# aws/karpenter-core

Measured on NVIDIA B200. Metric: pods scheduled/sec (Scheduler.Solve), higher is better.
Workload: dtype int64

## Files before the change

karpenter-core_b200/csrc/ksched.cu:

```cuda
#include <cuda_runtime.h>
#include <nccl.h>
#include <stdint.h>

#include <algorithm>
#include <chrono>
#include <cstdio>
#include <cstdlib>
#include <cstring>
#include <cub/cub.cuh>
#include <string>
#include <mutex>
#include <vector>

#include "ksched.h"
#include "reqmask.cuh"
#include "launch.cuh"

using ksched::KeyMeta;
using ksched::Req;

#define CUDA_TRY(h, expr)                                                                         \
  do {                                                                                            \
    cudaError_t _e = (expr);                                                                      \
    if (_e != cudaSuccess) {                                                                      \
// ... 697 lines not shown
        for (uint32_t f = g.filter_begin; f < g.filter_end && f < (uint32_t)pb->n_filter_terms; ++f)
          if (((pb->filter_terms[f].meta >> KSCHED_META_PRESENT_SHIFT) & 0xFFFF) == 0) x.has_filter = 0;
        x.max_skew = g.max_skew; x.host_row = host_row[ct.group];
        relx[e] = x;
      }
      CUDA_TRY(h, upload_vec(h, h->d_relx, relx));
    }
    CUDA_TRY(h, upload_vec(h, h->d_grp_host_total0, host_total));
    CUDA_TRY(h, upload_vec(h, h->d_grp_cnt0, cnt));
    CUDA_TRY(h, upload_vec(h, h->d_grp_registered0, registered));
    CUDA_TRY(h, h->d_grp_host0.ensure((size_t)std::max(nh, 1) * stride));
    CUDA_TRY(h, cudaMemsetAsync(h->d_grp_host0.ptr, 0, (size_t)std::max(nh, 1) * stride * sizeof(uint16_t), h->stream));
    if (NE > 0 && nh > 0) {
      CUDA_TRY(h, cudaMemcpy2DAsync(h->d_grp_host0.ptr, stride * sizeof(uint16_t), host.data(), (size_t)NE * sizeof(uint16_t), (size_t)NE * sizeof(uint16_t),
                                    (size_t)nh, cudaMemcpyHostToDevice, h->stream));
      h->tm.h2d_bytes += (int64_t)nh * NE * 2;
    }
    CUDA_TRY(h, cudaStreamSynchronize(h->stream));
    CUDA_TRY(h, h->d_grp_host_total.ensure(std::max(NG, 1)));
    CUDA_TRY(h, h->d_grp_cnt.ensure((size_t)std::max(NG, 1) * 64));
    CUDA_TRY(h, h->d_grp_registered.ensure(std::max(NG, 1)));
    CUDA_TRY(h, h->d_grp_host.ensure((size_t)std::max(nh, 1) * stride));
  }
  const size_t p1 = (size_t)std::max(P, 1);
  CUDA_TRY(h, h->d_order.ensure(p1)); CUDA_TRY(h, h->d_idx_tmp.ensure(p1)); CUDA_TRY(h, h->d_pod_pos.ensure(p1));
  CUDA_TRY(h, h->d_k_cpu.ensure(p1)); CUDA_TRY(h, h->d_k_mem.ensure(p1)); CUDA_TRY(h, h->d_k_tie.ensure(p1)); CUDA_TRY(h, h->d_k_tmp.ensure(p1));
  CUDA_TRY(h, h->d_rows.ensure(p1 * KSCHED_ROW_WORDS));
  CUDA_TRY(h, h->d_F.ensure(p1 * V * W32));
  CUDA_TRY(h, h->d_best.ensure(p1));
  CUDA_TRY(h, h->d_Fclass.ensure((size_t)std::max(NC, 1) * V * W32));
  CUDA_TRY(h, h->d_best_class.ensure((size_t)std::max(NC, 1)));
  CUDA_TRY(h, h->d_relax.ensure(p1)); CUDA_TRY(h, h->d_assign.ensure(p1)); CUDA_TRY(h, h->d_place_seq.ensure(p1));
  CUDA_TRY(h, h->d_queue.ensure(p1 + 1)); CUDA_TRY(h, h->d_last_len.ensure(p1)); CUDA_TRY(h, h->d_last_epoch.ensure(p1));
  const size_t mn = (size_t)MAXN;
  CUDA_TRY(h, h->d_nn_tmpl.ensure(mn)); CUDA_TRY(h, h->d_nn_count.ensure(mn)); CUDA_TRY(h, h->d_nn_tb.ensure(mn));
  CUDA_TRY(h, h->d_nn_req.ensure(8 * mn)); CUDA_TRY(h, h->d_nn_req_present.ensure(mn));
  CUDA_TRY(h, h->d_nn_vals.ensure(16 * mn)); CUDA_TRY(h, h->d_nn_meta.ensure(mn));
  CUDA_TRY(h, h->d_nn_opts.ensure((size_t)W32 * mn)); CUDA_TRY(h, h->d_nn_hp.ensure(mn));
  CUDA_TRY(h, h->d_ov_key.ensure(mn)); CUDA_TRY(h, h->d_ov_q.ensure(4 * mn)); CUDA_TRY(h, h->d_ov_bound.ensure(4 * mn)); CUDA_TRY(h, h->d_ov_bound2.ensure(4 * mn));
  CUDA_TRY(h, h->d_ov_node.ensure(mn)); CUDA_TRY(h, h->d_ov_flags.ensure(mn));
  CUDA_TRY(h, h->d_ov_absorbed.ensure(mn)); CUDA_TRY(h, h->d_ov_rejected.ensure(mn));
  {
    const size_t nfc = (size_t)std::max(NC, 1) * V;
    CUDA_TRY(h, h->d_fc_state.ensure(nfc)); CUDA_TRY(h, h->d_fc_dom.ensure(nfc)); CUDA_TRY(h, h->d_fc_front_state.ensure(nfc)); CUDA_TRY(h, h->d_fc_bound.ensure(nfc * 4)); CUDA_TRY(h, h->d_fc_bound2.ensure(nfc * 4));
    CUDA_TRY(h, h->d_fc_opts.ensure(nfc * W32));
    CUDA_TRY(h, h->d_fc_vals.ensure(nfc * KSCHED_MAX_KEYS)); CUDA_TRY(h, h->d_fc_meta.ensure(nfc)); CUDA_TRY(h, h->d_fc_q.ensure(nfc * KSCHED_MAX_RES));
    CUDA_TRY(h, h->d_fc_qp.ensure(nfc));
    const size_t nfd = kFreshMemoSlots;
    CUDA_TRY(h, h->d_fd_state.ensure(nfd)); CUDA_TRY(h, h->d_fd_dom.ensure(nfd)); CUDA_TRY(h, h->d_fd_fc.ensure(nfd)); CUDA_TRY(h, h->d_fd_meta.ensure(nfd));
    CUDA_TRY(h, h->d_fd_vals.ensure(nfd * KSCHED_MAX_KEYS)); CUDA_TRY(h, h->d_fd_opts.ensure(nfd * W32));
    CUDA_TRY(h, h->d_fd_bound.ensure(nfd * 4)); CUDA_TRY(h, h->d_fd_bound2.ensure(nfd * 4));
  }
  CUDA_TRY(h, h->d_remaining.ensure((size_t)V * KSCHED_MAX_RES));
  CUDA_TRY(h, h->d_counters.ensure(48));
  {
    size_t need = 0, n2 = 0;
    cub::DeviceRadixSort::SortPairs(nullptr, need, (uint64_t*)nullptr, (uint64_t*)nullptr, (uint32_t*)nullptr, (uint32_t*)nullptr, (int)p1, 0, 64, h->stream);
    n2 = need;
    CUDA_TRY(h, h->d_cub_tmp.ensure(n2 + 256));
    h->cub_tmp_bytes = n2 + 256;
  }
  CUDA_TRY(h, cudaStreamSynchronize(h->stream));
  h->uploaded = true;
  h->sorted = false;
  return KSCHED_OK;
}

static int run_sort(ksched_handle* h) {
  const int P = h->n_pods;
  if (P == 0) return KSCHED_OK;
  const int threads = 256, blocks = (P + threads - 1) / threads;
  if (h->sort1_bits > 0) {
    sort_key1_kernel<<<blocks, threads, 0, h->stream>>>(P, h->d_cls_rank.ptr, h->d_pod_class.ptr, h->d_ts.ptr, h->d_uid_rank.ptr, h->sort1_ts_min,
                                                        h->sort1_ts_bits, h->sort1_uid_bits, h->d_k_tie.ptr, h->d_idx_tmp.ptr);
    size_t tmp1 = h->cub_tmp_bytes;
    CUDA_TRY(h, cub::DeviceRadixSort::SortPairs(h->d_cub_tmp.ptr, tmp1, h->d_k_tie.ptr, h->d_k_tmp.ptr, h->d_idx_tmp.ptr, h->d_order.ptr, P, 0, h->sort1_bits,
                                                h->stream));
    const int gblocks1 = std::min((P + 7) / 8, 148 * 8);
    gather_rows_kernel<<<gblocks1, 256, 0, h->stream>>>(P, h->d_classes.ptr, h->d_pod_class.ptr, h->d_order.ptr, h->d_rows.ptr);
    h->tm.sort_launches = 3;
    h->sorted = true;
    return KSCHED_OK;
  }
  sort_keys_kernel<<<blocks, threads, 0, h->stream>>>(P, h->d_classes.ptr, h->d_pod_class.ptr, h->d_ts.ptr, h->d_uid_rank.ptr, h->d_k_cpu.ptr,
                                                      h->d_k_mem.ptr, h->d_k_tie.ptr, h->d_order.ptr);
  size_t tmp = h->cub_tmp_bytes;
  uint32_t *ia = h->d_order.ptr, *ib = h->d_idx_tmp.ptr;
  CUDA_TRY(h, cub::DeviceRadixSort::SortPairs(h->d_cub_tmp.ptr, tmp, h->d_k_tie.ptr, h->d_k_tmp.ptr, ia, ib, P, 0, 64, h->stream));
  gather_u64_kernel<<<blocks, threads, 0, h->stream>>>(P, h->d_k_mem.ptr, ib, h->d_k_tie.ptr);
  tmp = h->cub_tmp_bytes;
  CUDA_TRY(h, cub::DeviceRadixSort::SortPairs(h->d_cub_tmp.ptr, tmp, h->d_k_tie.ptr, h->d_k_tmp.ptr, ib, ia, P, 0, 64, h->stream));
  gather_u64_kernel<<<blocks, threads, 0, h->stream>>>(P, h->d_k_cpu.ptr, ia, h->d_k_tie.ptr);
  tmp = h->cub_tmp_bytes;
  CUDA_TRY(h, cub::DeviceRadixSort::SortPairs(h->d_cub_tmp.ptr, tmp, h->d_k_tie.ptr, h->d_k_tmp.ptr, ia, ib, P, 0, 64, h->stream));
  CUDA_TRY(h, cudaMemcpyAsync(h->d_order.ptr, ib, (size_t)P * sizeof(uint32_t), cudaMemcpyDeviceToDevice, h->stream));
  const int gblocks = std::min((P + 7) / 8, 148 * 8);
  gather_rows_kernel<<<gblocks, 256, 0, h->stream>>>(P, h->d_classes.ptr, h->d_pod_class.ptr, h->d_order.ptr, h->d_rows.ptr);
  h->tm.sort_launches = 7;
  h->sorted = true;
  return KSCHED_OK;
}

static void fill_k1(ksched_handle* h, K1Params& k1) {
  k1.cat = h->cat;
  k1.rows = reinterpret_cast<const uint64_t*>(h->d_classes.ptr);
  k1.n_pods = h->n_classes;
  k1.itype_sets = h->d_itype_sets.ptr;
// ... 64 lines not shown
  if (h->n_pods == 0) return KSCHED_OK;
  const int RW = h->cat.n_templates * h->cat.W32;
  const int nblk = (h->n_pods + 31) / 32;
  const int blocks = std::max(1, std::min(148 * 8, (nblk + 7) / 8));
  feasibility_kernel<<<blocks, 256, 0, h->stream>>>(h->d_rows.ptr, h->n_pods, h->n_classes, RW, h->d_Fclass.ptr, h->d_best_class.ptr, h->d_F.ptr,
                                                    h->d_best.ptr);
  CUDA_TRY(h, cudaGetLastError());
  h->tm.feasibility_launches = 2;
  const long long C = (long long)h->cat.n_templates * h->cat.n_types;
  h->tm.feasibility_bytes = (long long)h->n_pods * 256 + C * 256 + (long long)h->n_pods * C / 8;
  return KSCHED_OK;
}

struct ResetSeg { void* dst; const void* src; unsigned long long bytes; };
struct ResetTable { int n; ResetSeg seg[30]; };
__global__ void reset_kernel(ResetTable t) {
  const size_t tid = (size_t)blockIdx.x * blockDim.x + threadIdx.x, nth = (size_t)gridDim.x * blockDim.x;
  for (int q = 0; q < t.n; ++q) {
    const ResetSeg sg = t.seg[q];
    const size_t n16 = sg.bytes / 16;
    uint4* d = static_cast<uint4*>(sg.dst);
    const uint4* sv = static_cast<const uint4*>(sg.src);
    for (size_t i = tid; i < n16; i += nth) d[i] = sv ? sv[i] : make_uint4(0, 0, 0, 0);
    unsigned char* db = static_cast<unsigned char*>(sg.dst);
    const unsigned char* sb = static_cast<const unsigned char*>(sg.src);
    for (size_t i = n16 * 16 + tid; i < sg.bytes; i += nth) db[i] = sb ? sb[i] : 0;
  }
}

static int reset_state(ksched_handle* h, const int64_t* d_remaining_src = nullptr, void* also_zero = nullptr, size_t also_zero_bytes = 0) {
  const int P = h->n_pods, NE = std::max(h->n_existing, 1), NG = std::max(h->n_groups, 1);
  CUDA_TRY(h, h->d_cls_cursor.ensure((size_t)std::max(h->n_classes, 1)));
  ResetTable t{};
  auto add = [&](void* dst, const void* src, size_t bytes) { if (bytes) t.seg[t.n++] = ResetSeg{dst, src, (unsigned long long)bytes}; };
  add(h->d_pod_class.ptr, h->d_pod_class0.ptr, (size_t)P * 4);
  add(h->d_relax.ptr, nullptr, (size_t)std::max(P, 1) * 4);
  add(h->d_ex_req.ptr, h->d_ex_req0.ptr, (size_t)8 * NE * 8);
  add(h->d_ex_req_present.ptr, h->d_ex_req_present0.ptr, (size_t)NE * 4);
  add(h->d_ex_vals.ptr, h->d_ex_vals0.ptr, (size_t)16 * NE * 8);
  add(h->d_ex_meta.ptr, h->d_ex_meta0.ptr, (size_t)NE * 8);
  add(h->d_ex_hp.ptr, h->d_ex_hp0.ptr, (size_t)NE * 8);
  add(h->d_ex_closed.ptr, nullptr, (size_t)NE);
  add(h->d_cls_cursor.ptr, nullptr, (size_t)std::max(h->n_classes, 1) * 4);
  if (h->have_volumes) add(h->d_ex_vol.ptr, h->d_ex_vol0.ptr, (size_t)h->n_existing * sizeof(ksched_node_volumes));
  add(h->d_grp_cnt.ptr, h->d_grp_cnt0.ptr, (size_t)NG * 64 * 4);
  add(h->d_grp_registered.ptr, h->d_grp_registered0.ptr, (size_t)NG * 8);
  add(h->d_grp_host_total.ptr, h->d_grp_host_total0.ptr, (size_t)NG * 4);
  add(h->d_grp_active.ptr, h->d_grp_active0.ptr, (size_t)NG);
  add(h->d_grp_min_slot.ptr, nullptr, (size_t)NG * 4);
  const size_t hs = (size_t)std::max(h->n_hostgroups, 1) * ((size_t)h->n_existing + h->max_new);
  add(h->d_grp_host.ptr, h->d_grp_host0.ptr, hs * 2);
  if (d_remaining_src)
    add(h->d_remaining.ptr, d_remaining_src, (size_t)h->cat.n_templates * KSCHED_MAX_RES * 8);
  add(h->d_counters.ptr, nullptr, 48 * sizeof(long long));
  add(h->d_fc_state.ptr, nullptr, (size_t)std::max(h->n_classes, 1) * h->cat.n_templates);
  add(h->d_fc_front_state.ptr, nullptr, (size_t)std::max(h->n_classes, 1) * h->cat.n_templates);
  add(h->d_fd_state.ptr, nullptr, (size_t)kFreshMemoSlots);
  add(also_zero, nullptr, also_zero_bytes);
  if (!d_remaining_src) {
    std::vector<int64_t> rem((size_t)h->cat.n_templates * KSCHED_MAX_RES);
    for (int v = 0; v < h->cat.n_templates; ++v)
      for (int r = 0; r < KSCHED_MAX_RES; ++r) rem[(size_t)v * KSCHED_MAX_RES + r] = h->h_templates[v].remaining[r];
    CUDA_TRY(h, cudaMemcpyAsync(h->d_remaining.ptr, rem.data(), rem.size() * 8, cudaMemcpyHostToDevice, h->stream));
    CUDA_TRY(h, cudaStreamSynchronize(h->stream));
  }
  reset_kernel<<<148 * 2, 256, 0, h->stream>>>(t);
  CUDA_TRY(h, cudaGetLastError());
  return KSCHED_OK;
}

static std::mutex g_k2_mu;
static cudaEvent_t g_k2_done[64] = {};

static int run_pack(ksched_handle* h) {
  K2Params& k2 = h->k2_host;
  k2.cat = h->cat;
  PackState& s = k2.st;
  s.relx = h->d_relx.ptr;
  s.classes = h->d_classes.ptr; s.groups = h->d_groups.ptr; s.class_topo = h->d_class_topo.ptr; s.filter_terms = h->d_filter_terms.ptr;
  s.itype_sets = h->d_itype_sets.ptr; s.itype_complement = h->d_itype_comp.ptr; s.hostname_reqs = h->d_hostname_reqs.ptr;
  s.order = h->d_order.ptr; s.rows = h->d_rows.ptr; s.F = h->d_F.ptr; s.best = h->d_best.ptr;
  s.pod_pos = h->d_pod_pos.ptr; s.use_F = h->world == 1 ? 1 : 0;
  s.n_pods = h->n_pods; s.n_classes = h->n_classes; s.n_existing = h->n_existing; s.n_groups = h->n_groups; s.max_new = h->max_new;
  for (int r = 0; r < KSCHED_MAX_RES; ++r) s.min_req[r] = h->min_req[r];
  s.pod_class = h->d_pod_class.ptr; s.relax_level = h->d_relax.ptr; s.assign = h->d_assign.ptr; s.place_seq = h->d_place_seq.ptr;
  s.queue = h->d_queue.ptr; s.last_len = h->d_last_len.ptr; s.last_epoch = h->d_last_epoch.ptr;
  s.ex_req = h->d_ex_req.ptr; s.ex_avail = h->d_ex_avail.ptr; s.ex_req_present = h->d_ex_req_present.ptr; s.ex_avail_present = h->d_ex_avail_present.ptr;
  s.ex_vals = h->d_ex_vals.ptr; s.ex_meta = h->d_ex_meta.ptr; s.ex_taintset = h->d_ex_taintset.ptr; s.ex_itype = h->d_ex_itype.ptr;
  s.ex_hp = h->d_ex_hp.ptr; s.ex_closed = h->d_ex_closed.ptr;
  s.cls_cursor = h->d_cls_cursor.ptr;
  s.cls_vol = h->have_volumes ? h->d_cls_vol.ptr : nullptr; s.ex_vol = h->have_volumes ? h->d_ex_vol.ptr : nullptr;
  for (int d = 0; d < KSCHED_MAX_VOLUME_DRIVERS; ++d) s.vol_mask[d] = h->vol_mask[d];
  s.nn_tmpl = h->d_nn_tmpl.ptr; s.nn_count = h->d_nn_count.ptr; s.nn_tb = h->d_nn_tb.ptr; s.nn_req = h->d_nn_req.ptr;
  s.nn_req_present = h->d_nn_req_present.ptr;
  s.nn_vals = h->d_nn_vals.ptr; s.nn_meta = h->d_nn_meta.ptr; s.nn_opts = h->d_nn_opts.ptr; s.nn_hp = h->d_nn_hp.ptr;
  s.ov_key = h->d_ov_key.ptr; s.ov_q = h->d_ov_q.ptr; s.ov_bound = h->d_ov_bound.ptr; s.ov_bound2 = h->d_ov_bound2.ptr; s.ov_node = h->d_ov_node.ptr; s.ov_flags = h->d_ov_flags.ptr;
  s.fc_state = h->d_fc_state.ptr; s.fc_opts = h->d_fc_opts.ptr; s.fc_bound = h->d_fc_bound.ptr; s.fc_bound2 = h->d_fc_bound2.ptr; s.fc_dom = h->d_fc_dom.ptr; s.fc_front_state = h->d_fc_front_state.ptr;
  s.fc_vals = h->d_fc_vals.ptr; s.fc_meta = h->d_fc_meta.ptr; s.fc_q = h->d_fc_q.ptr; s.fc_qp = h->d_fc_qp.ptr;
  s.ov_absorbed = h->d_ov_absorbed.ptr; s.ov_rejected = h->d_ov_rejected.ptr;
  s.fd_cap = kFreshMemoSlots; s.fd_state = h->d_fd_state.ptr; s.fd_fc = h->d_fd_fc.ptr; s.fd_meta = h->d_fd_meta.ptr; s.fd_vals = h->d_fd_vals.ptr;
  s.fd_opts = h->d_fd_opts.ptr; s.fd_bound = h->d_fd_bound.ptr; s.fd_bound2 = h->d_fd_bound2.ptr; s.fd_dom = h->d_fd_dom.ptr;
  s.count_visited = h->count_visited;
  s.stop_new_nodes = h->stop_new_nodes;
  s.grp_cnt = h->d_grp_cnt.ptr; s.grp_registered = h->d_grp_registered.ptr; s.grp_host = h->d_grp_host.ptr;
  s.grp_host_row = h->d_grp_host_row.ptr; s.grp_host_total = h->d_grp_host_total.ptr; s.remaining = h->d_remaining.ptr;
  s.grp_active = h->d_grp_active.ptr; s.grp_min_slot = h->d_grp_min_slot.ptr;
  s.counters = h->d_counters.ptr;
// ... 60 lines not shown
    ncclResult_t r = ncclAllReduce(h->d_best.ptr, h->d_best.ptr, (size_t)h->n_pods, ncclUint64, ncclMin, h->comm, h->stream);
    if (r != ncclSuccess) { h->err = std::string("ncclAllReduce: ") + ncclGetErrorString(r); return KSCHED_ERR_NCCL; }
  }
  CUDA_TRY(h, cudaEventRecord(h->ev[3], h->stream));
  if ((rc = run_pack(h)) != KSCHED_OK) return rc;
  CUDA_TRY(h, cudaEventRecord(h->ev[4], h->stream));
  CUDA_TRY(h, cudaStreamSynchronize(h->stream));
  CUDA_TRY(h, cudaGetLastError());
  h->tm.sort_us = ev_us(h->ev[0], h->ev[1]);
  h->tm.feasibility_us = ev_us(h->ev[1], h->ev[2]);
  h->tm.allreduce_us = ev_us(h->ev[2], h->ev[3]);
  h->tm.pack_us = ev_us(h->ev[3], h->ev[4]);
  h->tm.total_us = ev_us(h->ev[0], h->ev[4]);
  return KSCHED_OK;
}

int ksched_run_feasibility_only(ksched_handle* h, int do_flush, float* elapsed_us) {
  if (!h || !h->uploaded) return KSCHED_ERR_INVALID;
  CUDA_TRY(h, cudaSetDevice(h->device));
  int rc;
  if (!h->sorted) {
    CUDA_TRY(h, cudaMemcpyAsync(h->d_pod_class.ptr, h->d_pod_class0.ptr, (size_t)h->n_pods * 4, cudaMemcpyDeviceToDevice, h->stream));
    if ((rc = run_sort(h)) != KSCHED_OK) return rc;
  }
  CUDA_TRY(h, cudaEventRecord(h->ev[7], h->stream));
  if ((rc = run_class_feasibility(h)) != KSCHED_OK) return rc;
  if (do_flush && (rc = flush_l2(h)) != KSCHED_OK) return rc;
  CUDA_TRY(h, cudaEventRecord(h->ev[5], h->stream));
  if ((rc = run_feasibility(h)) != KSCHED_OK) return rc;
  CUDA_TRY(h, cudaEventRecord(h->ev[6], h->stream));
  CUDA_TRY(h, cudaStreamSynchronize(h->stream));
  CUDA_TRY(h, cudaGetLastError());
  if (elapsed_us) *elapsed_us = ev_us(h->ev[5], h->ev[6]);
  h->tm.feasibility_us = ev_us(h->ev[5], h->ev[6]);
  h->tm.class_feasibility_us = ev_us(h->ev[7], h->ev[5]);
  return KSCHED_OK;
}

#ifdef KSCHED_PROFILE_PACK
static void print_pack_profile(const long long* counters) {
  fprintf(stderr, "[pack profile] generic: topo=%lld existing=%lld eval=%lld commit=%lld fresh=%lld fail=%lld | fastblock=%lld genericcall=%lld | "
                  "n_generic=%lld inflight_placed=%lld fresh_steps=%lld failures=%lld paths[rej,cached,row,dyn,cachedempty]=%lld,%lld,%lld,%lld,%lld steps=%lld\n",
          counters[8], counters[9], counters[10], counters[11], counters[12], counters[13], counters[14], counters[15], counters[17], counters[18],
          counters[19], counters[20], counters[21], counters[22], counters[23], counters[24], counters[25], counters[5]);
  fprintf(stderr, "[pack profile] fresh: decide=%lld words=%lld commit=%lld rest=%lld | in-flight verify=%lld\n", counters[26], counters[27], counters[28],
          counters[12], counters[29]);
  fprintf(stderr, "[pack profile] in-flight commit: winner+barrier=%lld record=%lld rest=%lld\n", counters[30], counters[31], counters[11]);
  fprintf(stderr, "[pack profile] class_run: calls=%lld pods=%lld bails=%lld ineligible=%lld cycles=%lld\n", counters[40], counters[41], counters[42], counters[43],
          counters[14]);
  fprintf(stderr, "[pack profile] mask run steps=%lld with >1 admissible domain=%lld round-able=%lld (counters shared with generic n/fresh: ignore there)\n", counters[18], counters[19], counters[17]);
  fprintf(stderr, "[pack profile] mask run: build cycles=%lld (refused %lld) loop cycles=%lld pods=%lld entries=%lld\n", counters[38], counters[47], counters[6], counters[7], counters[16]);
  fprintf(stderr, "[pack profile] class_run without mask-key spread: cycles=%lld pods=%lld level+fill iterations=%lld (fill %lld) fresh=%lld per-pod=%lld | with: cycles=%lld pods=%lld fresh=%lld per-pod=%lld\n",
          counters[32], counters[33], counters[34], counters[46], counters[35], counters[44], counters[36], counters[37], counters[39], counters[45]);
}
#endif

int ksched_download(ksched_handle* h, const ksched_problem* pb, ksched_result* res) {
  if (!h || !pb || !res || !h->uploaded) return KSCHED_ERR_INVALID;
  CUDA_TRY(h, cudaSetDevice(h->device));
  const int P = h->n_pods, NE = h->n_existing, MAXN = h->max_new, W32 = h->cat.W32, W64 = h->W64, V = h->cat.n_templates;
  long long counters[48];
  CUDA_TRY(h, cudaMemcpyAsync(counters, h->d_counters.ptr, sizeof counters, cudaMemcpyDeviceToHost, h->stream));
  CUDA_TRY(h, cudaStreamSynchronize(h->stream));
#ifdef KSCHED_PROFILE_PACK
  print_pack_profile(counters);
#endif
  if (counters[4] != 0) {
    h->err = counters[4] == KSCHED_ERR_OVERFLOW ? "new-node capacity exceeded" : "a pod is constrained by more topology groups than the kernel supports";
    return (int)counters[4];
  }
  const int n_new = (int)counters[0];
  h->tm.d2h_bytes = (int64_t)sizeof counters + (int64_t)P * 4 * ((res->assign != nullptr) + (res->relax_level != nullptr) + (res->place_seq != nullptr)) +
                    (int64_t)n_new * (1 + 4 + 4 + 8 + 64 + 128 + (int64_t)W32 * 4) + (res->existing_reqs ? (int64_t)NE * 136 : 0) +
                    (res->launch ? (int64_t)n_new * (int64_t)sizeof(ksched_launch_choice) : 0) +
                    (res->feasibility ? (int64_t)P * V * W32 * 4 + (int64_t)P * 4 : 0) + (res->best_column ? (int64_t)P * 12 : 0);
  res->n_new_nodes = n_new;
  res->n_unscheduled = (int)counters[1];
  res->nodes_visited = counters[2];
  res->add_calls = counters[3];
  h->tm.pack_steps = counters[5];
  if (res->assign) CUDA_TRY(h, cudaMemcpyAsync(res->assign, h->d_assign.ptr, (size_t)P * 4, cudaMemcpyDeviceToHost, h->stream));
  if (res->relax_level) CUDA_TRY(h, cudaMemcpyAsync(res->relax_level, h->d_relax.ptr, (size_t)P * 4, cudaMemcpyDeviceToHost, h->stream));
  if (res->place_seq) CUDA_TRY(h, cudaMemcpyAsync(res->place_seq, h->d_place_seq.ptr, (size_t)P * 4, cudaMemcpyDeviceToHost, h->stream));
  if (n_new > 0 && res->new_nodes && res->new_node_types) {
    std::vector<uint8_t> tmpl(n_new);
    std::vector<int32_t> count(n_new);
    std::vector<int64_t> req((size_t)8 * n_new);
    std::vector<uint32_t> reqp(n_new), opts((size_t)W32 * n_new);
    std::vector<uint64_t> vals((size_t)16 * n_new), meta(n_new);
    CUDA_TRY(h, cudaMemcpyAsync(tmpl.data(), h->d_nn_tmpl.ptr, n_new, cudaMemcpyDeviceToHost, h->stream));
    CUDA_TRY(h, cudaMemcpyAsync(count.data(), h->d_nn_count.ptr, (size_t)n_new * 4, cudaMemcpyDeviceToHost, h->stream));
    CUDA_TRY(h, cudaMemcpyAsync(reqp.data(), h->d_nn_req_present.ptr, (size_t)n_new * 4, cudaMemcpyDeviceToHost, h->stream));
    CUDA_TRY(h, cudaMemcpyAsync(meta.data(), h->d_nn_meta.ptr, (size_t)n_new * 8, cudaMemcpyDeviceToHost, h->stream));
    CUDA_TRY(h, cudaMemcpy2DAsync(req.data(), (size_t)n_new * 8, h->d_nn_req.ptr, (size_t)MAXN * 8, (size_t)n_new * 8, 8, cudaMemcpyDeviceToHost, h->stream));
    CUDA_TRY(h, cudaMemcpy2DAsync(vals.data(), (size_t)n_new * 8, h->d_nn_vals.ptr, (size_t)MAXN * 8, (size_t)n_new * 8, 16, cudaMemcpyDeviceToHost, h->stream));
    CUDA_TRY(h, cudaMemcpy2DAsync(opts.data(), (size_t)n_new * 4, h->d_nn_opts.ptr, (size_t)MAXN * 4, (size_t)n_new * 4, W32, cudaMemcpyDeviceToHost, h->stream));
    CUDA_TRY(h, cudaStreamSynchronize(h->stream));
    for (int n = 0; n < n_new; ++n) {
      ksched_new_node& o = res->new_nodes[n];
      std::memset(&o, 0, sizeof o);
      o.template_index = tmpl[n];
      o.pod_count = count[n];
      o.requests_present = reqp[n];
      for (int r = 0; r < 8; ++r) o.requests[r] = req[(size_t)r * n_new + n];
      for (int k = 0; k < 16; ++k) o.reqs.values[k] = vals[(size_t)k * n_new + n];
      o.reqs.meta = meta[n];
      uint32_t* dst = reinterpret_cast<uint32_t*>(res->new_node_types + (size_t)n * W64);
      for (int w = 0; w < W32; ++w) dst[w] = opts[(size_t)w * n_new + n];
      if (W32 & 1) dst[W32] = 0;
    }
  }
  if (res->launch && n_new > 0) {
    if (!h->cat.offer_keys) { h->err = "ksched_result.launch needs ksched_catalog.offering_keys"; return KSCHED_ERR_INVALID; }
    CUDA_TRY(h, h->d_launch.ensure((size_t)n_new));
// ... 255 lines not shown
```

karpenter-core_b200/csrc/pack_kernel.cuh:

```cuda
#pragma once

namespace {

constexpr int kActCap = 1280;
constexpr int kHotRes = 4;

struct HotSmem {
  unsigned long long key[kActCap];
  long long q[kHotRes][kActCap];
  long long bound[kHotRes][kActCap];
  long long bound2[kHotRes][kActCap];
  int node[kActCap];
  unsigned short flags[kActCap];
  unsigned absorbed[kActCap];
  unsigned rejected[kActCap];
  unsigned long long nn_last[kActCap];
};

struct Hot {
  HotSmem* sm;
  unsigned long long* ov_key;
  long long* ov_q;
  long long* ov_bound;
  long long* ov_bound2;
// ... 1170 lines not shown
    io->add_calls = add_calls;
  }
}

constexpr int kRunHost = 4;
constexpr int kRunMask = 2;
constexpr int kRunDom = 16;
constexpr int kTopoCap = 768;
constexpr int kRunVariants = 4;
constexpr int kRunW32 = 64;
constexpr int kRunWarps = kPackThreads / 32;
constexpr int kRunChunk = 128;
constexpr unsigned kRoomSlow = 0xFFFFu, kRoomMax = 0x7FFEu, kRpDead = 0x80000000u;
constexpr size_t kRunArrayBytes = (size_t)kTopoCap * (kRunMask * 4 + kRunHost * 2) + (size_t)kActCap * 4;

struct RunVariant {
  uint32_t opts[kRunW32];
  uint64_t vals[KSCHED_MAX_KEYS];
  uint64_t meta;
  long long q[KSCHED_MAX_RES];
  long long b1[kHotRes], b2[kHotRes];
  uint32_t qp;
  uint32_t rp;
  unsigned short fl;
  uint8_t dom[kRunMask];
};
struct RunCtx {
  uint32_t cls;
  int eligible;
  int n_host, n_mask, n_var, var_next;
  int tomb;
  int h_row[kRunHost], h_group[kRunHost], h_lim[kRunHost];
  int h_inc[kRunHost];
  uint8_t h_times[kRunHost];
  int m_group[kRunMask], m_skew[kRunMask];
  uint8_t m_key[kRunMask], m_self[kRunMask], m_rec[kRunMask], m_wk[kRunMask];
  uint32_t m_registered[kRunMask], m_neutral[kRunMask], m_tallow[kRunMask];
  int32_t cnt[kRunWarps][kRunMask][kRunDom];
  unsigned long long red_key[2][32];
  unsigned red_pay[2][32];
  uint32_t q_pod[2][kRunChunk], q_cls[2][kRunChunk];
  int32_t q_node[2][kRunChunk];
  int q_end[2];
  int lv_cnt[2];
  int lv_fill[2];
  RunVariant var[kRunVariants];
};
__shared__ RunCtx g_rc;

constexpr int kM1Dom = 8;
constexpr int kM1Lists = kM1Dom + 1;
constexpr int kM1Lv = 12;
constexpr uint16_t kM1None = 0xFFFF;
struct M1Ctx {
  uint16_t tl[kM1Lv][kM1Lists];
  uint16_t head[kM1Lists];
  uint16_t ap[kM1Lv][kM1Lists];
  uint16_t ae[kM1Lv][kM1Lists];
  int bcnt[kM1Lv * kM1Lists];
  int bad;
  int out_adv, out_reason, out_tick, out_n_new, out_n_active;
  int n_fresh;
  uint32_t fr[kRunChunk];
};
__shared__ M1Ctx g_m1;

struct RunIO {
  int qi, head, qlen, tick, seq, n_active, n_new, parity;
  long long add_calls;
  int placed;
  int status;
  int fresh_valid, fresh_a;
  uint32_t fresh_cls;
};
__shared__ RunIO g_rio;

__device__ __forceinline__ int run_pick(uint32_t cand, const int32_t* cn) {
  int d = __ffs(cand) - 1;
  cand &= cand - 1;
  int32_t best = cn[d];
  while (cand) {
    const int e = __ffs(cand) - 1;
    cand &= cand - 1;
    if (cn[e] < best) { best = cn[e]; d = e; }
  }
  return d;
}
__device__ __noinline__ unsigned run_room(const HotSmem* hs, int a, const long long* req, uint32_t res, int RH) {
  const unsigned short fl = hs->flags[a];
  const uint32_t qp = ((fl >> 1) & 0xF) | res;
  long long best = 0;
  bool inexact_ok = true;
  for (int f = 0; f < 2; ++f) {
    if (f == 1 && !(fl & kFlTwo)) break;
    long long rf = kRoomMax;
    for (int r = 0; r < RH; ++r) {
      if (!((qp >> r) & 1)) continue;
      const long long slack = (f ? hs->bound2[r][a] : hs->bound[r][a]) - hs->q[r][a];
      if (req[r] > 0) {
        const long long k = slack < req[r] ? 0 : slack / req[r];
        rf = k < rf ? k : rf;
      } else if (slack < 0) rf = 0;
    }
    if (f == 0) inexact_ok = rf > 0;
    best = rf > best ? rf : best;
  }
// ... 351 lines not shown
            int lv = La - 1;
            while (m1.tl[lv][L] == kM1None) --lv;
            const int pred = m1.tl[lv][L];
            m1_nxt[a] = m1_nxt[pred];
            m1_nxt[pred] = (uint16_t)a;
            if (m1.tl[La][L] == kM1None) m1.tl[La][L] = (uint16_t)a;
            if (pred == h) { n1 = a; nk = ak; nr = ar; }
            if (pred == tcur) { bn = a; bnc = La; }
          }
        };
        auto insert_back1 = [&](int a, unsigned long long ak, uint32_t ar) {
          const int hl = h >= 0 ? (int)(hk >> 32) : 0x7fffffff;
          if (hl > 1) {
            m1_nxt[a] = h >= 0 ? (uint16_t)h : kM1None;
            m1.tl[1][L] = (uint16_t)a;
            tcur = a; bn = h; bnc = hl;
            n1 = h; nk = hk; nr = hr;
            h = a; hk = ak; hr = ar;
          } else if (hl == 1) {
            m1_nxt[a] = bn >= 0 ? (uint16_t)bn : kM1None;
            m1_nxt[tcur] = (uint16_t)a;
            m1.tl[1][L] = (uint16_t)a;
            if (tcur == h) { n1 = a; nk = ak; nr = ar; }
            tcur = a;
          } else {
            int lv = 1;
            while (m1.tl[lv][L] == kM1None) --lv;
            const int pred = m1.tl[lv][L];
            m1_nxt[a] = m1_nxt[pred];
            m1_nxt[pred] = (uint16_t)a;
            m1.tl[1][L] = (uint16_t)a;
            if (pred == h) { n1 = a; nk = ak; nr = ar; }
            if (pred == tcur) { bn = a; bnc = 1; }
          }
        };
        auto pop_head = [&](int c) {
          h = n1; hk = nk; hr = nr;
          n1 = -1; nk = ~0ull; nr = 0;
          if (h >= 0) {
            n1 = nxt_of(h);
            if (n1 >= 0) { nk = hs->key[n1]; nr = rpv[n1]; }
          }
          if (h < 0 || (int)(hk >> 32) != c) {
            m1.tl[c][L] = kM1None;
            level_state();
          }
        };
        const bool rounds = m_rec0 && m_bias0 == 0;
        int li = i, ltick = tick, lnew = n_new, lact = n_active, nfr = 0;
        int i_end = rc.q_end[buf];
        if (i + qlen < i_end) i_end = i + qlen;
        int reason = 0;
        const int slack = m_bias0 < -(1 << 30) ? (1 << 30) : -m_bias0;
        while (li < i_end) {
          const int mn = __reduce_min_sync(FULL, valid ? cnt_d : INT32_MAX);
          const bool allowed = valid && cnt_d - mn <= slack;
          const unsigned okm = __ballot_sync(FULL, allowed);
          const bool cand_ok = L < kM1Dom ? allowed : (L == kM1Dom && okm != 0);
          const unsigned long long key = cand_ok ? hk : ~0ull;
          const unsigned long long wkey = warp_min_u64(key);
#ifdef KSCHED_PROFILE_PACK
          {
            const unsigned have = __ballot_sync(FULL, L < kM1Dom && allowed && h >= 0);
            const unsigned long long ukey = __shfl_sync(FULL, hk, kM1Dom);
            unsigned long long mx = (L < kM1Dom && allowed && h >= 0) ? hk : 0ull;
            for (int o = 16; o; o >>= 1) { const unsigned long long t = __shfl_xor_sync(FULL, mx, o); mx = t > mx ? t : mx; }
            const int na = __popc(okm);
            if (L == 0 && na > 1 && have == okm && ukey > mx && i_end - li >= na) s.counters[17] += 1;
            if (L == 0) s.counters[18] += 1;
            if (L == 0 && na > 1) s.counters[19] += 1;
          }
#endif
          if (rounds) {
            const int na = __popc(okm);
            if (na > 1 && i_end - li >= na) {
              const bool act = L < kM1Dom && allowed;
              const bool hd = act && h >= 0;
              const unsigned hv = __ballot_sync(FULL, hd), fv = okm & ~hv;
              const bool bad_l = hd && ((hr & 0xFFFF) == kRoomSlow || (int)(hk >> 32) + 1 >= kM1Lv);
              const unsigned long long ukey = __shfl_sync(FULL, hk, kM1Dom);
              const unsigned hi = hd ? (unsigned)(hk >> 32) : 0u;
              const unsigned mhi = __reduce_max_sync(FULL, hi);
              const unsigned mlo = __reduce_max_sync(FULL, (hd && hi == mhi) ? (unsigned)hk : 0u);
              const unsigned long long mx = ((unsigned long long)mhi << 32) | mlo;
              int vi_l = -1;
              const int nf = __popc(fv);
              bool fresh_ok = true;
              if (fv) {
                const bool fl = act && h < 0;
                if (fl) for (int v2 = 0; v2 < rc.n_var && vi_l < 0; ++v2) if (rc.var[v2].dom[0] == L) vi_l = v2;
                fresh_ok = ukey == ~0ull && (fv & ~rc.m_tallow[0]) == 0 && !__any_sync(FULL, fl && vi_l < 0) && lnew + nf <= MAXN &&
                           lact + nf <= kActCap && lact + nf <= kTopoCap;
                for (int j = 0; j < n_host; ++j) fresh_ok = fresh_ok && rc.h_lim[j] >= 0;
              }
              if (fresh_ok && !__any_sync(FULL, bad_l) && (hv == 0 || ukey > mx)) {
                int rank = 0;
                for (unsigned m = hv; m; m &= m - 1) {
                  const unsigned long long k2 = __shfl_sync(FULL, hk, __ffs(m) - 1);
                  rank += k2 < hk;
                }
                bool closed_l = false;
                if (hd) {
                  const int a = h;
                  const uint32_t rp = hr;
                  const int c = (int)(hk >> 32);
                  const int mytick = ltick + rank;
                  pop_head(c);
// ... 8 lines not shown
                  const unsigned long long nkey = order_key(c + 1, -(mytick + 1));
                  unsigned long long skey = nkey;
                  rc.q_node[buf][li + rank] = -(a + 2);
                  if ((rp2 & 0xFFFF) == 0) {
                    const int placed = (rp2 >> 16) & 0x7FFF;
                    long long nq[kHotRes], cb1[kHotRes], cb2[kHotRes];
#pragma unroll
                    for (int r = 0; r < kHotRes; ++r) { nq[r] = hs->q[r][a] + placed * p_req[r]; cb1[r] = hs->bound[r][a]; cb2[r] = hs->bound2[r][a]; }
                    const unsigned short fl = (unsigned short)(hs->flags[a] | ((p_res & 0xF) << 1));
                    if (node_closed(nq, min_req, RH, cb1, cb2, fl)) {
                      skey = ~0ull;
                      hs->nn_last[a] = ((unsigned long long)(unsigned)(c + 1) << 32) | (unsigned)(-(mytick + 1));
                      closed_l = true;
                    }
                  }
                  hs->key[a] = skey;
                  rpv[a] = rp2;
                  if ((rp2 & 0xFFFF) != 0 && !(rp2 & kRpDead)) insert_front(a, c + 1, nkey, rp2);
                  ++cnt_d;
                } else if (act) {
                  const RunVariant& v = rc.var[vi_l];
                  const int idx = __popc(fv & ((1u << L) - 1u));
                  const int n = lnew + idx, a = lact + idx;
                  const int mytick = ltick + __popc(hv) + idx;
                  for (int j = 0; j < n_host; ++j) {
                    const int times = rc.h_times[j];
                    hc[j * kTopoCap + a] = (uint16_t)times;
                    if (times) s.grp_host[(size_t)rc.h_row[j] * hstride + NE + n] = (uint16_t)times;
                  }
                  const unsigned long long fkey = order_key(1, mytick + 1);
                  hs->key[a] = fkey;
#pragma unroll
                  for (int r = 0; r < kHotRes; ++r) { hs->q[r][a] = v.q[r]; hs->bound[r][a] = v.b1[r]; hs->bound2[r][a] = v.b2[r]; }
                  hs->node[a] = n;
                  hs->flags[a] = v.fl;
                  hs->absorbed[a] = simple ? cls : KSCHED_NONE;
                  hs->rejected[a] = KSCHED_NONE;
                  rpv[a] = v.rp;
                  rc.q_node[buf][li + __popc(hv) + idx] = NE + n;
                  zv[a] = (1u << L) | (3u << 16);
                  m1.fr[nfr + idx] = (uint32_t)a | ((uint32_t)vi_l << 16);
                  if ((v.rp & 0xFFFF) != 0 && !(v.rp & kRpDead)) insert_back1(a, fkey, v.rp);
                  ++cnt_d;
                }
                if (nf && L < n_host && rc.h_times[L]) rc.h_inc[L] = rc.h_inc[L] + nf;
                const unsigned tb = __ballot_sync(FULL, closed_l);
                if (L == 0 && tb) rc.tomb = rc.tomb + __popc(tb);
                lnew += nf;
                lact += nf;
                nfr += nf;
                ltick += na;
                li += na;
                __syncwarp();
                continue;
              }
            }
          }
          if (wkey != ~0ull) {
            const int wl = __ffs(__ballot_sync(FULL, key == wkey)) - 1;
            const int a = __shfl_sync(FULL, h, wl);
            const uint32_t rp = __shfl_sync(FULL, hr, wl);
            if ((rp & 0xFFFF) == kRoomSlow) { reason = 1; break; }
            int d = wl;
            const bool pin = wl == kM1Dom;
            if (pin) {
              const int mc = __reduce_min_sync(FULL, allowed ? cnt_d : INT32_MAX);
              d = __ffs(__ballot_sync(FULL, allowed && cnt_d == mc)) - 1;
              if (!((rc.m_neutral[0] >> d) & 1) || !((zv[a] & (1u << 17)) || rc.m_wk[0])) { reason = 1; break; }
            }
            const int c = (int)(wkey >> 32);
            if (L == wl) pop_head(c);
            uint32_t rp2 = rp - 1 + (1u << 16);
            bool dead_l = false;
            if (L < n_host) {
              const int times = rc.h_times[L];
              const int old = hc[L * kTopoCap + a];
              const int now = old + times > 0xFFFF ? 0xFFFF : old + times;
              if (times) hc[L * kTopoCap + a] = (uint16_t)now;
              dead_l = now > rc.h_lim[L];
            }
            if (n_host > 0 && __any_sync(FULL, dead_l)) rp2 |= kRpDead;
            const unsigned long long nkey = order_key(c + 1, -(ltick + 1));
            if (L == 0) {
              unsigned long long skey = nkey;
              if (pin) {
                const int n = hs->node[a], k = rc.m_key[0];
                zv[a] = (1u << d) | (3u << 16);
                s.nn_vals[(size_t)k * MAXN + n] = 1ull << d;
                atomicOr(reinterpret_cast<unsigned long long*>(&s.nn_meta[n]), 1ull << (KSCHED_META_PRESENT_SHIFT + k));
                atomicAnd(reinterpret_cast<unsigned long long*>(&s.nn_meta[n]), ~(1ull << (KSCHED_META_COMPLEMENT_SHIFT + k)));
              }
              rc.q_node[buf][li] = -(a + 2);
              if ((rp2 & 0xFFFF) == 0) {
                const int placed = (rp2 >> 16) & 0x7FFF;
                long long nq[kHotRes], cb1[kHotRes], cb2[kHotRes];
#pragma unroll
                for (int r = 0; r < kHotRes; ++r) { nq[r] = hs->q[r][a] + placed * p_req[r]; cb1[r] = hs->bound[r][a]; cb2[r] = hs->bound2[r][a]; }
                const unsigned short fl = (unsigned short)(hs->flags[a] | ((p_res & 0xF) << 1));
                if (node_closed(nq, min_req, RH, cb1, cb2, fl)) {
                  skey = ~0ull;
                  hs->nn_last[a] = ((unsigned long long)(unsigned)(c + 1) << 32) | (unsigned)(-(ltick + 1));
                  rc.tomb = rc.tomb + 1;
                }
              }
              hs->key[a] = skey;
              rpv[a] = rp2;
            }
            if ((rp2 & 0xFFFF) != 0 && !(rp2 & kRpDead)) {
              if (c + 1 >= kM1Lv) reason = 2;
              else if (L == d) insert_front(a, c + 1, nkey, rp2);
            }
            if (m_rec0 && L == d) ++cnt_d;
            ++ltick;
            ++li;
            __syncwarp();
            if (reason == 2) break;
          } else {
            if (lnew >= MAXN || lact >= kActCap || lact >= kTopoCap || rc.n_var == 0) { reason = 1; break; }
            bool ok = true;
            for (int j = 0; j < n_host; ++j) ok = ok && rc.h_lim[j] >= 0;
            const unsigned cand = rc.m_tallow[0] & okm;
            if (!ok || !cand) { reason = 1; break; }
            const bool in_c = (cand >> L) & 1;
            const int mc = __reduce_min_sync(FULL, in_c ? cnt_d : INT32_MAX);
            const int fd = __ffs(__ballot_sync(FULL, in_c && cnt_d == mc)) - 1;
            int vi = -1;
            for (int v2 = 0; v2 < rc.n_var && vi < 0; ++v2) if (rc.var[v2].dom[0] == fd) vi = v2;
            if (vi < 0) { reason = 1; break; }
            const RunVariant& v = rc.var[vi];
            const int n = lnew, a = lact;
            if (L < n_host) {
              const int times = rc.h_times[L];
              hc[L * kTopoCap + a] = (uint16_t)times;
              if (times) {
                s.grp_host[(size_t)rc.h_row[L] * hstride + NE + n] = (uint16_t)times;
                rc.h_inc[L] = rc.h_inc[L] + 1;
              }
            }
            const unsigned long long fkey = order_key(1, ltick + 1);
            if (L == 0) {
              hs->key[a] = fkey;
#pragma unroll
              for (int r = 0; r < kHotRes; ++r) { hs->q[r][a] = v.q[r]; hs->bound[r][a] = v.b1[r]; hs->bound2[r][a] = v.b2[r]; }
              hs->node[a] = n;
              hs->flags[a] = v.fl;
              hs->absorbed[a] = simple ? cls : KSCHED_NONE;
              hs->rejected[a] = KSCHED_NONE;
              rpv[a] = v.rp;
              rc.q_node[buf][li] = NE + n;
              zv[a] = (1u << fd) | (3u << 16);
              m1.fr[nfr] = (uint32_t)a | ((uint32_t)vi << 16);
            }
            ++nfr;
            if (L == fd) {
              if ((v.rp & 0xFFFF) != 0 && !(v.rp & kRpDead)) insert_back1(a, fkey, v.rp);
              if (m_rec0) ++cnt_d;
            }
            ++ltick; ++lnew; ++lact; ++li;
            __syncwarp();
          }
        }
        __syncwarp();
        if (L < kM1Dom) for (int w = 0; w < nwarps; ++w) rc.cnt[w][0][L] = cnt_d;
        if (L < kM1Lists) m1.head[L] = h >= 0 ? (uint16_t)h : kM1None;
        if (L == 0) { m1.out_adv = li - i; m1.out_reason = reason; m1.out_tick = ltick; m1.out_n_new = lnew; m1.out_n_active = lact; m1.n_fresh = nfr; }
      }
      __syncthreads();
      {
        const int nfr = m1.n_fresh;
        for (int e = tid; e < nfr * 64; e += T) {
          const uint32_t rec = m1.fr[e >> 6];
          const int a = (int)(rec & 0xFFFF), w = e & 63;
          const RunVariant& v = rc.var[rec >> 16];
          const int n = hs->node[a];
          if (w < W32) s.nn_opts[(size_t)w * MAXN + n] = v.opts[w];
          if (w < c.n_keys) s.nn_vals[(size_t)w * MAXN + n] = v.vals[w];
          if (w < KSCHED_MAX_RES) s.nn_req[(size_t)w * MAXN + n] = v.q[w];
          if (w == 0) {
            s.nn_meta[n] = v.meta;
            s.nn_tmpl[n] = (uint8_t)(v.fl >> 8);
            s.nn_req_present[n] = v.qp;
            s.nn_hp[n] = 0;
            if (((rpv[a] >> 16) & 0x7FFF) == 0) {
              s.nn_count[n] = 1;
              s.nn_tb[n] = (int)((unsigned)hs->key[a] ^ 0x80000000u);
            }
          }
        }
      }
      const int m_adv = m1.out_adv, m_reason = m1.out_reason;
      tick = m1.out_tick; n_new = m1.out_n_new; n_active = m1.out_n_active;
      qi += m_adv;
      qlen -= m_adv;
      __syncthreads();
#ifdef KSCHED_PROFILE_PACK
      if (tid == 0) { s.counters[6] += clock64() - m1_t1; s.counters[7] += m_adv; s.counters[16] += 1; }
#endif
      if (m_reason == 1) { status = 1; break; }
      if (qlen == 0) break;
      if (m_reason == 2) m1_ok = false;
      continue;
    }
    if (lvl && n_active > 0 && n_active <= 32 && s.use_level_warp) {
      if (warp == 0) {
        const unsigned FULL = 0xffffffffu;
        const int a = lane;
        const bool mine = a < n_active;
        int li = i, ltick = tick, reason = 0;
        int i_end = rc.q_end[buf];
        if (i + qlen < i_end) i_end = i + qlen;
        while (li < i_end) {
          const uint32_t rp = mine ? rpv[a] : 0u;
          const unsigned long long key = mine ? hs->key[a] : ~0ull;
          const bool el = mine && (rp & 0xFFFF) != 0 && !(rp & kRpDead);
// ... 725 lines not shown
```

Measured before the change: 2.074 million.

## Batch unpinned-list placements into warp-wide rounds in mask run loop

```diff
diff --git a/karpenter-core_b200/csrc/ksched.cu b/karpenter-core_b200/csrc/ksched.cu
--- a/karpenter-core_b200/csrc/ksched.cu
+++ b/karpenter-core_b200/csrc/ksched.cu
@@ -773,7 +773,7 @@
     CUDA_TRY(h, h->d_fd_bound.ensure(nfd * 4)); CUDA_TRY(h, h->d_fd_bound2.ensure(nfd * 4));
   }
   CUDA_TRY(h, h->d_remaining.ensure((size_t)V * KSCHED_MAX_RES));
-  CUDA_TRY(h, h->d_counters.ensure(48));
+  CUDA_TRY(h, h->d_counters.ensure(80));
   {
     size_t need = 0, n2 = 0;
     cub::DeviceRadixSort::SortPairs(nullptr, need, (uint64_t*)nullptr, (uint64_t*)nullptr, (uint32_t*)nullptr, (uint32_t*)nullptr, (int)p1, 0, 64, h->stream);
@@ -944,7 +944,7 @@
   add(h->d_grp_host.ptr, h->d_grp_host0.ptr, hs * 2);
   if (d_remaining_src)
     add(h->d_remaining.ptr, d_remaining_src, (size_t)h->cat.n_templates * KSCHED_MAX_RES * 8);
-  add(h->d_counters.ptr, nullptr, 48 * sizeof(long long));
+  add(h->d_counters.ptr, nullptr, 80 * sizeof(long long));
   add(h->d_fc_state.ptr, nullptr, (size_t)std::max(h->n_classes, 1) * h->cat.n_templates);
   add(h->d_fc_front_state.ptr, nullptr, (size_t)std::max(h->n_classes, 1) * h->cat.n_templates);
   add(h->d_fd_state.ptr, nullptr, (size_t)kFreshMemoSlots);
@@ -1111,6 +1111,13 @@
   fprintf(stderr, "[pack profile] mask run: build cycles=%lld (refused %lld) loop cycles=%lld pods=%lld entries=%lld\n", counters[38], counters[47], counters[6], counters[7], counters[16]);
   fprintf(stderr, "[pack profile] class_run without mask-key spread: cycles=%lld pods=%lld level+fill iterations=%lld (fill %lld) fresh=%lld per-pod=%lld | with: cycles=%lld pods=%lld fresh=%lld per-pod=%lld\n",
           counters[32], counters[33], counters[34], counters[46], counters[35], counters[44], counters[36], counters[37], counters[39], counters[45]);
+  static const char* kinds[6] = {"round pinned", "round fresh", "round unpinned", "single pinned", "single pin", "single fresh"};
+  for (int k = 0; k < 6; ++k)
+    fprintf(stderr, "[pack profile] mask run %-14s: iterations=%lld pods=%lld cycles=%lld\n", kinds[k], counters[48 + 3 * k], counters[49 + 3 * k],
+            counters[50 + 3 * k]);
+  fprintf(stderr, "[pack profile] mask run declined rounds: na<=1=%lld staged<na=%lld unpinned-first=%lld room-slow=%lld level=%lld no-fresh=%lld "
+                  "unpinned-few=%lld unpinned-pin=%lld\n",
+          counters[66], counters[67], counters[68], counters[69], counters[70], counters[71], counters[72], counters[73]);
 }
 #endif
 
@@ -1118,7 +1125,7 @@
   if (!h || !pb || !res || !h->uploaded) return KSCHED_ERR_INVALID;
   CUDA_TRY(h, cudaSetDevice(h->device));
   const int P = h->n_pods, NE = h->n_existing, MAXN = h->max_new, W32 = h->cat.W32, W64 = h->W64, V = h->cat.n_templates;
-  long long counters[48];
+  long long counters[80];
   CUDA_TRY(h, cudaMemcpyAsync(counters, h->d_counters.ptr, sizeof counters, cudaMemcpyDeviceToHost, h->stream));
   CUDA_TRY(h, cudaStreamSynchronize(h->stream));
 #ifdef KSCHED_PROFILE_PACK
diff --git a/karpenter-core_b200/csrc/pack_kernel.cuh b/karpenter-core_b200/csrc/pack_kernel.cuh
--- a/karpenter-core_b200/csrc/pack_kernel.cuh
+++ b/karpenter-core_b200/csrc/pack_kernel.cuh
@@ -1246,6 +1246,8 @@
 constexpr int kM1Lists = kM1Dom + 1;
 constexpr int kM1Lv = 12;
 constexpr uint16_t kM1None = 0xFFFF;
+constexpr int kM1Win = 16;
+static_assert(kM1Win > kM1Dom && kM1Win + kM1Dom + 1 < 32, "the unpinned window needs its own lanes");
 struct M1Ctx {
   uint16_t tl[kM1Lv][kM1Lists];
   uint16_t head[kM1Lists];
@@ -1703,7 +1705,17 @@
         if (i + qlen < i_end) i_end = i + qlen;
         int reason = 0;
         const int slack = m_bias0 < -(1 << 30) ? (1 << 30) : -m_bias0;
+#ifdef KSCHED_PROFILE_PACK
+#define M1_KIND(k, pods) { if (L == 0) { s.counters[48 + 3 * (k)] += 1; s.counters[49 + 3 * (k)] += (pods); s.counters[50 + 3 * (k)] += clock64() - it_t0; } }
+#define M1_DECLINE(r) { if (L == 0) s.counters[66 + (r)] += 1; }
+#else
+#define M1_KIND(k, pods) {}
+#define M1_DECLINE(r) {}
+#endif
         while (li < i_end) {
+#ifdef KSCHED_PROFILE_PACK
+          const long long it_t0 = clock64();
+#endif
           const int mn = __reduce_min_sync(FULL, valid ? cnt_d : INT32_MAX);
           const bool allowed = valid && cnt_d - mn <= slack;
           const unsigned okm = __ballot_sync(FULL, allowed);
@@ -1818,9 +1830,125 @@
                 ltick += na;
                 li += na;
                 __syncwarp();
+                M1_KIND(nf ? 1 : 0, na)
                 continue;
               }
-            }
+              if (ukey != ~0ull && !(hv == okm && ukey > mx)) {
+                const int u0 = __shfl_sync(FULL, h, kM1Dom), u1 = __shfl_sync(FULL, n1, kM1Dom);
+                int us = L == kM1Win ? u0 : (L == kM1Win + 1 ? u1 : -1);
+                int cur = u1;
+                for (int j = 2; j <= na + 1; ++j) {
+                  cur = cur >= 0 ? nxt_of(cur) : -1;
+                  if (L == kM1Win + j) us = cur;
+                }
+                unsigned long long uk = ~0ull;
+                uint32_t ur = 0;
+                if (us >= 0) { uk = hs->key[us]; ur = rpv[us]; }
+                const bool un = L >= kM1Win && L < kM1Win + na && us >= 0;
+                const bool cnd = hd || un;
+                const unsigned long long ck = hd ? hk : uk;
+                const unsigned cm = __ballot_sync(FULL, cnd);
+                int pos = 0;
+                for (unsigned m = cm; m; m &= m - 1) pos += __shfl_sync(FULL, ck, __ffs(m) - 1) < ck;
+                const unsigned long long code = cnd ? (unsigned long long)(un ? 8 : L) << (4 * pos) : 0ull;
+                const unsigned long long desc = ((unsigned long long)__reduce_or_sync(FULL, (unsigned)(code >> 32)) << 32) |
+                                                __reduce_or_sync(FULL, (unsigned)code);
+                unsigned open = okm;
+                unsigned long long asg = 0;
+                int ju = 0;
+                for (int p = 0, nc = __popc(cm); p < nc && open; ++p) {
+                  const int cd = (int)(desc >> (4 * p)) & 15;
+                  const int d = cd == 8 ? __ffs(open) - 1 : cd;
+                  if ((open >> d) & 1) {
+                    asg |= (unsigned long long)(0x80 | (cd == 8 ? 0x40 | ju << 3 : 0) | (na - __popc(open))) << (8 * d);
+                    open &= ~(1u << d);
+                  }
+                  ju += cd == 8;
+                }
+                const unsigned b = L < kM1Dom ? (unsigned)(asg >> (8 * L)) & 0xFF : 0u;
+                const int src = (b & 0x40) ? kM1Win + ((b >> 3) & 7) : L;
+                const int ua = __shfl_sync(FULL, us, src);
+                const unsigned long long uka = __shfl_sync(FULL, uk, src);
+                const uint32_t ura = __shfl_sync(FULL, ur, src);
+                const bool mine = (b & 0x80) != 0, pin = (b & 0x40) != 0;
+                const int rank = b & 7, a = pin ? ua : h;
+                const uint32_t rp = pin ? ura : hr;
+                const int c = (int)((pin ? uka : hk) >> 32);
+                bool bad_m = mine && ((rp & 0xFFFF) == kRoomSlow || c + 1 >= kM1Lv);
+                if (pin) bad_m = bad_m || !((rc.m_neutral[0] >> L) & 1) || !((zv[a] & (1u << 17)) || rc.m_wk[0]);
+#ifdef KSCHED_PROFILE_PACK
+                if (open) M1_DECLINE(6)
+                else if (__any_sync(FULL, bad_m)) M1_DECLINE(7)
+#endif
+                if (open == 0 && !__any_sync(FULL, bad_m)) {
+                  bool closed_l = false;
+                  if (mine) {
+                    const int mytick = ltick + rank;
+                    if (!pin) pop_head(c);
+                    uint32_t rp2 = rp - 1 + (1u << 16);
+                    for (int j = 0; j < n_host; ++j) {
+                      const int times = rc.h_times[j];
+                      const int old = hc[j * kTopoCap + a];
+                      const int now = old + times > 0xFFFF ? 0xFFFF : old + times;
+                      if (times) hc[j * kTopoCap + a] = (uint16_t)now;
+                      if (now > rc.h_lim[j]) rp2 |= kRpDead;
+                    }
+                    const unsigned long long nkey = order_key(c + 1, -(mytick + 1));
+                    unsigned long long skey = nkey;
+                    rc.q_node[buf][li + rank] = -(a + 2);
+                    if (pin) {
+                      const int n = hs->node[a], k = rc.m_key[0];
+                      zv[a] = (1u << L) | (3u << 16);
+                      s.nn_vals[(size_t)k * MAXN + n] = 1ull << L;
+                      atomicOr(reinterpret_cast<unsigned long long*>(&s.nn_meta[n]), 1ull << (KSCHED_META_PRESENT_SHIFT + k));
+                      atomicAnd(reinterpret_cast<unsigned long long*>(&s.nn_meta[n]), ~(1ull << (KSCHED_META_COMPLEMENT_SHIFT + k)));
+                    }
+                    if ((rp2 & 0xFFFF) == 0) {
+                      const int placed = (rp2 >> 16) & 0x7FFF;
+                      long long nq[kHotRes], cb1[kHotRes], cb2[kHotRes];
+#pragma unroll
+                      for (int r = 0; r < kHotRes; ++r) { nq[r] = hs->q[r][a] + placed * p_req[r]; cb1[r] = hs->bound[r][a]; cb2[r] = hs->bound2[r][a]; }
+                      const unsigned short fl = (unsigned short)(hs->flags[a] | ((p_res & 0xF) << 1));
+                      if (node_closed(nq, min_req, RH, cb1, cb2, fl)) {
+                        skey = ~0ull;
+                        hs->nn_last[a] = ((unsigned long long)(unsigned)(c + 1) << 32) | (unsigned)(-(mytick + 1));
+                        closed_l = true;
+                      }
+                    }
+                    hs->key[a] = skey;
+                    rpv[a] = rp2;
+                    if ((rp2 & 0xFFFF) != 0 && !(rp2 & kRpDead)) insert_front(a, c + 1, nkey, rp2);
+                    ++cnt_d;
+                  }
+                  const int nh = __shfl_sync(FULL, us, kM1Win + ju), nn = __shfl_sync(FULL, us, kM1Win + ju + 1);
+                  const unsigned long long nhk = __shfl_sync(FULL, uk, kM1Win + ju), nnk = __shfl_sync(FULL, uk, kM1Win + ju + 1);
+                  const uint32_t nhr = __shfl_sync(FULL, ur, kM1Win + ju), nnr = __shfl_sync(FULL, ur, kM1Win + ju + 1);
+                  const unsigned long long uk_nx = __shfl_down_sync(FULL, uk, 1);
+                  const bool emptied = L >= kM1Win && L < kM1Win + ju && (uk_nx >> 32) != (uk >> 32);
+                  if (emptied) m1.tl[(int)(uk >> 32)][kM1Dom] = kM1None;
+                  const bool any_emptied = __any_sync(FULL, emptied);
+                  if (L == kM1Dom) { h = nh; hk = nhk; hr = nhr; n1 = nn; nk = nnk; nr = nnr; }
+                  if (any_emptied) {
+                    __syncwarp();
+                    if (L == kM1Dom) level_state();
+                  }
+                  const unsigned tb = __ballot_sync(FULL, closed_l);
+                  if (L == 0 && tb) rc.tomb = rc.tomb + __popc(tb);
+                  ltick += na;
+                  li += na;
+                  __syncwarp();
+                  M1_KIND(2, na)
+                  continue;
+                }
+              }
+#ifdef KSCHED_PROFILE_PACK
+              else if (ukey != ~0ull && hv != 0 && ukey <= mx) M1_DECLINE(2)
+              else if (__any_sync(FULL, bad_l && (hr & 0xFFFF) == kRoomSlow)) M1_DECLINE(3)
+              else if (__any_sync(FULL, bad_l)) M1_DECLINE(4)
+              else M1_DECLINE(5)
+#endif
+            } else if (na <= 1) M1_DECLINE(0)
+            else M1_DECLINE(1)
           }
           if (wkey != ~0ull) {
             const int wl = __ffs(__ballot_sync(FULL, key == wkey)) - 1;
@@ -1880,6 +2008,7 @@
             ++ltick;
             ++li;
             __syncwarp();
+            M1_KIND(pin ? 4 : 3, 1)
             if (reason == 2) break;
           } else {
             if (lnew >= MAXN || lact >= kActCap || lact >= kTopoCap || rc.n_var == 0) { reason = 1; break; }
@@ -1924,8 +2053,11 @@
             }
             ++ltick; ++lnew; ++lact; ++li;
             __syncwarp();
-          }
-        }
+            M1_KIND(5, 1)
+          }
+        }
+#undef M1_KIND
+#undef M1_DECLINE
         __syncwarp();
         if (L < kM1Dom) for (int w = 0; w < nwarps; ++w) rc.cnt[w][0][L] = cnt_d;
         if (L < kM1Lists) m1.head[L] = h >= 0 ? (uint16_t)h : kM1None;
```

New measurement: 2.158 million (median of 6 runs). +4.1%, better.
